# jpreprocess/jbonsai

Measured on AMD Instinct MI355X. Metric: 48 kHz PCM samples/sec (whole node), batched utterances, higher is better.
Workload: dtype f64

## Files before the change

### include/jbonsai_amd.h

```cpp
#ifndef JBONSAI_AMD_H
#define JBONSAI_AMD_H

#include <stddef.h>
#include <stdint.h>

#ifdef __cplusplus
extern "C" {
#endif

#define JB_MAX_STREAM 3
#define JB_MAX_WINDOW 8
#define JB_NODATA (-1e10)

typedef enum jb_status {
    JB_OK = 0,
    JB_ERR_INVALID = -1,
    JB_ERR_UNSUPPORTED = -2,
    JB_ERR_DEVICE = -3,
    JB_ERR_MODEL = -4,
    JB_ERR_LABEL = -5,
    JB_ERR_PARSE_OPTION = -6,
    JB_ERR_WEIGHT = -7,
    JB_ERR_BUFFER = -8
} jb_status;
// ... 94 lines not shown
int jb_batch_create_indexed(const jb_voice_desc *voice, const jb_pdf_set *set, const jb_index_utt *utts,
                            size_t n_utts, const jb_batch_opts *opts, jb_batch **out);
typedef struct jb_utt_voc {
    double alpha, beta, volume;
} jb_utt_voc;
int jb_batch_create_voc(const jb_voice_desc *voice, const jb_state_utt *utts, size_t n_utts, const jb_utt_voc *voc,
                        const jb_batch_opts *opts, jb_batch **out);
int jb_batch_create_indexed_voc(const jb_voice_desc *voice, const jb_pdf_set *set, const jb_index_utt *utts,
                                size_t n_utts, const jb_utt_voc *voc, const jb_batch_opts *opts, jb_batch **out);
int jb_batch_run(jb_batch *b);
int jb_batch_sync(jb_batch *b);
int jb_batch_run_timed(jb_batch *b, float *total_ms, float *vocoder_ms);
int jb_batch_last_timing(jb_batch *b, float *total_ms, float *vocoder_ms);
size_t jb_batch_size(const jb_batch *b);
size_t jb_batch_num_frames(const jb_batch *b, size_t utt);
size_t jb_batch_num_samples(const jb_batch *b, size_t utt);
size_t jb_batch_total_samples(const jb_batch *b);
int jb_batch_read_pcm(jb_batch *b, size_t utt, double *dst, size_t cap);
int jb_batch_read_pcm_i16(jb_batch *b, size_t utt, int16_t *dst, size_t cap);
int jb_batch_read_pcm_all(jb_batch *b, double *const *dst);
int jb_batch_read_pcm_i16_all(jb_batch *b, int16_t *const *dst);
int jb_batch_read_track(jb_batch *b, size_t utt, uint32_t stream, double *dst, size_t cap);
int jb_release_cached_memory(void);
int jb_set_cached_memory_limit(size_t megabytes);
int jb_batch_read_coefficients(jb_batch *b, size_t utt, double *dst, size_t cap);
int jb_batch_read_first_coefficients(jb_batch *b, size_t utt, double *dst, size_t cap);
int jb_batch_read_excitation(jb_batch *b, size_t utt, double *dst, size_t cap);
void *jb_batch_device_pcm(jb_batch *b, size_t *n_samples);
size_t jb_batch_pcm_offset(const jb_batch *b, size_t utt);
int jb_batch_info(const jb_batch *b, uint32_t *chunk_frames, uint32_t *warmup_frames,
                  uint32_t *n_items, uint32_t *n_redo);
int jb_batch_redo_stats(const jb_batch *b, uint32_t *n_partial, uint32_t *n_full);
int jb_batch_kernel_info(const jb_batch *b, uint32_t *lane_triple, uint32_t *waves_per_simd);
uint32_t jb_batch_gang_fallbacks(const jb_batch *b);
int jb_batch_set_output_rate(jb_batch *b, const uint32_t *out_hz, size_t n);
uint32_t jb_batch_output_rate(const jb_batch *b, size_t utt);
int jb_batch_read_pcm_native(jb_batch *b, size_t utt, double *dst, size_t cap);
int jb_batch_set_loudness_target(jb_batch *b, const double *target_lufs, size_t n, double ceiling_dbfs);
int jb_batch_loudness(jb_batch *b, size_t utt, double *lufs, double *peak_dbfs, double *gain_db);
void jb_batch_free(jb_batch *b);

int jb_paramgen_vocode_batch(const jb_voice_desc *voice, const jb_state_utt *utts, size_t n_utts,
                             const jb_batch_opts *opts, double *const *pcm, size_t *n_samples);

int jb_mlpg_batch(const jb_voice_desc *voice, const jb_state_utt *utts, size_t n_utts, const jb_batch_opts *opts,
                  double *const *tracks, size_t *n_frames);

typedef struct jb_track_utt {
    size_t n_spectrum, n_lf0, n_lpf;
    uint32_t spectrum_width, lf0_width, lpf_width;
    uint32_t reserved;
    const double *spectrum;
    const double *lf0;
    const double *lpf;
} jb_track_utt;
int jb_batch_create_from_tracks(const jb_voice_desc *voice, const jb_track_utt *utts, size_t n_utts,
                                const jb_batch_opts *opts, jb_batch **out);
int jb_vocode_tracks_batch(const jb_voice_desc *voice, const jb_track_utt *utts, size_t n_utts,
                           const jb_batch_opts *opts, double *const *pcm, size_t *n_samples);
int jb_vocoder_synthesize_batch(const jb_voice_desc *voice, const jb_track_utt *utts, size_t n_utts,
                                const jb_batch_opts *opts, double *const *pcm, size_t *n_samples);

int jb_resample_filter(uint32_t in_hz, uint32_t out_hz, uint32_t *L, uint32_t *M, uint32_t *ntaps, double *taps,
                       size_t cap);
int jb_resample_pcm_batch(const double *const *in, const size_t *n_in, size_t n, uint32_t in_hz, uint32_t out_hz,
                          int32_t device, double **out, size_t *n_out);
// ... 162 lines not shown
```

### jbonsai_amd/_ffi.py

```python
from __future__ import annotations

import ctypes as C
import subprocess
from pathlib import Path

_HERE = Path(__file__).resolve().parent
LIB_PATH = _HERE / "libjbonsai_amd.so"

MAX_STREAM = 3
MAX_WINDOW = 8
NODATA = -1e10

JB_OK = 0
ERRORS = {
    -1: "JB_ERR_INVALID", -2: "JB_ERR_UNSUPPORTED", -3: "JB_ERR_DEVICE", -4: "JB_ERR_MODEL",
    -5: "JB_ERR_LABEL", -6: "JB_ERR_PARSE_OPTION", -7: "JB_ERR_WEIGHT", -8: "JB_ERR_BUFFER",
}
BATCH_KEEP_TRACKS = 1
BATCH_GENERIC_MLPG = 2
BATCH_SERIAL = 4
BATCH_WAVE_KERNEL = 8
BATCH_LANE_KERNEL = 16
BATCH_SERIAL_GV = 32
BATCH_PCM_I16 = 64
# ... 75 lines not shown


class IndexUtt(C.Structure):
    _fields_ = [
        ("num_states", C.c_uint32),
        ("durations", C.POINTER(C.c_uint32)),
        ("stream", IndexStream * MAX_STREAM),
        ("lf0_offset", C.c_double),
    ]


class TrackUtt(C.Structure):
    _fields_ = [
        ("n_spectrum", C.c_size_t), ("n_lf0", C.c_size_t), ("n_lpf", C.c_size_t),
        ("spectrum_width", C.c_uint32), ("lf0_width", C.c_uint32), ("lpf_width", C.c_uint32),
        ("reserved", C.c_uint32),
        ("spectrum", C.POINTER(C.c_double)), ("lf0", C.POINTER(C.c_double)), ("lpf", C.POINTER(C.c_double)),
    ]


class UttVoc(C.Structure):
    _fields_ = [("alpha", C.c_double), ("beta", C.c_double), ("volume", C.c_double)]


class BatchOpts(C.Structure):
    _fields_ = [("device", C.c_int32), ("flags", C.c_uint32), ("chunk_frames", C.c_uint32),
                ("warmup_frames", C.c_uint32), ("verify_tol", C.c_double), ("reserved0", C.c_uint32), ("reserved", C.c_uint32)]


SYMBOLS = [
    "jb_batch_create", "jb_batch_run", "jb_batch_sync", "jb_batch_run_timed", "jb_batch_last_timing", "jb_batch_size",
    "jb_batch_num_frames", "jb_batch_num_samples", "jb_batch_total_samples", "jb_batch_read_pcm",
    "jb_batch_read_pcm_i16", "jb_batch_read_pcm_all", "jb_batch_read_pcm_i16_all", "jb_pdf_set_create", "jb_pdf_set_free", "jb_batch_create_indexed", "jb_batch_read_track", "jb_release_cached_memory", "jb_set_cached_memory_limit", "jb_batch_read_coefficients", "jb_batch_read_first_coefficients", "jb_batch_read_excitation", "jb_batch_device_pcm", "jb_batch_pcm_offset",
    "jb_batch_info", "jb_batch_kernel_info", "jb_batch_redo_stats", "jb_batch_gang_fallbacks", "jb_batch_free", "jb_paramgen_vocode_batch",
    "jb_mlpg_batch", "jb_batch_create_from_tracks", "jb_vocode_tracks_batch",
    "jb_engine_load", "jb_engine_load_from_bytes", "jb_engine_new", "jb_engine_free",
    "jb_engine_set_sampling_frequency", "jb_engine_get_sampling_frequency",
    "jb_engine_set_fperiod", "jb_engine_get_fperiod", "jb_engine_set_volume", "jb_engine_get_volume",
    "jb_engine_set_msd_threshold", "jb_engine_get_msd_threshold", "jb_engine_set_gv_weight",
    "jb_engine_get_gv_weight", "jb_engine_set_phoneme_alignment_flag",
    "jb_engine_get_phoneme_alignment_flag", "jb_engine_set_batch_invariant", "jb_engine_get_batch_invariant",
    "jb_engine_set_fast_invariant", "jb_engine_get_fast_invariant",
    "jb_engine_set_speed", "jb_engine_get_speed",
    "jb_engine_set_alpha", "jb_engine_get_alpha", "jb_engine_set_beta", "jb_engine_get_beta",
    "jb_engine_set_additional_half_tone", "jb_engine_get_additional_half_tone",
    "jb_engine_num_voices", "jb_engine_num_streams", "jb_engine_num_states",
    "jb_engine_set_interpolation_weight", "jb_engine_get_interpolation_weight", "jb_synthesize", "jb_pcm_free", "jb_write_wav_i16", "jb_write_wav_f64", "jb_synthesize_batch", "jb_synthesize_batch_i16", "jb_pcm_i16_free",
    "jb_engine_model_shape", "jb_engine_pdf_table", "jb_engine_tree_index",
    "jb_engine_states", "jb_states_utt", "jb_engine_voice_desc", "jb_states_free",
    "jb_generator_new", "jb_generator_new_from_tracks", "jb_vocoder_synthesize_batch", "jb_generator_fperiod", "jb_generator_synthesized_frames",
    "jb_generator_total_frames", "jb_generator_step", "jb_generator_step_n", "jb_generator_free",
    "jb_comm_unique_id", "jb_comm_init", "jb_comm_rank", "jb_comm_size", "jb_comm_free", "jb_gather_pcm",
    "jb_gathered_samples", "jb_gathered_sample_bytes", "jb_gathered_device", "jb_gathered_read", "jb_gathered_free",
    "jb_lpt_partition", "jb_paramgen_vocode_batch_multi", "jb_synthesize_batch_multi", "jb_synthesize_batch_i16_multi",
    "jb_states_duration_params", "jb_last_error", "jb_device_count", "jb_device_arch", "jb_device_pci_bus_id", "jb_version", "jb_default_verify_tol",
    "jb_batch_create_voc", "jb_batch_create_indexed_voc", "jb_synthesize_batch_each", "jb_synthesize_batch_each_i16",
    "jb_batch_set_output_rate", "jb_batch_output_rate", "jb_batch_read_pcm_native", "jb_resample_filter",
    "jb_resample_pcm_batch", "jb_engine_set_output_sampling_frequency", "jb_engine_get_output_sampling_frequency",
    "jb_batch_set_loudness_target", "jb_batch_loudness", "jb_loudness_filter", "jb_loudness_pcm_batch",
    "jb_engine_set_loudness_target", "jb_engine_get_loudness_target", "jb_engine_set_peak_ceiling",
    "jb_engine_get_peak_ceiling",
]


def build(force: bool = False) -> Path:
    srcs = list((_HERE / "csrc").glob("*.hip")) + list((_HERE / "csrc").glob("*.cpp")) + \
        list((_HERE / "csrc").glob("*.h")) + [_HERE.parent / "include" / "jbonsai_amd.h"]
# ... 27 lines not shown
                                  C.POINTER(vp)]
    L.jb_pdf_set_create.argtypes = [C.POINTER(PdfTable), C.c_uint32, C.c_uint32, C.c_int32, C.POINTER(vp)]
    L.jb_pdf_set_free.argtypes = [vp]
    L.jb_pdf_set_free.restype = None
    L.jb_batch_create_indexed.argtypes = [C.POINTER(VoiceDesc), vp, C.POINTER(IndexUtt), sz, C.POINTER(BatchOpts),
                                          C.POINTER(vp)]
    L.jb_batch_create_voc.argtypes = [C.POINTER(VoiceDesc), C.POINTER(StateUtt), sz, C.POINTER(UttVoc),
                                      C.POINTER(BatchOpts), C.POINTER(vp)]
    L.jb_batch_create_indexed_voc.argtypes = [C.POINTER(VoiceDesc), vp, C.POINTER(IndexUtt), sz, C.POINTER(UttVoc),
                                              C.POINTER(BatchOpts), C.POINTER(vp)]
    L.jb_batch_run.argtypes = [vp]
    L.jb_batch_sync.argtypes = [vp]
    L.jb_batch_run_timed.argtypes = [vp, C.POINTER(C.c_float), C.POINTER(C.c_float)]
    L.jb_batch_last_timing.argtypes = [vp, C.POINTER(C.c_float), C.POINTER(C.c_float)]
    for n in ("jb_batch_size", "jb_batch_total_samples"):
        getattr(L, n).restype = sz
        getattr(L, n).argtypes = [vp]
    for n in ("jb_batch_num_frames", "jb_batch_num_samples", "jb_batch_pcm_offset"):
        getattr(L, n).restype = sz
        getattr(L, n).argtypes = [vp, sz]
    L.jb_batch_read_pcm.argtypes = [vp, sz, vp, sz]
    L.jb_batch_read_pcm_all.argtypes = [vp, C.POINTER(vp)]
    L.jb_batch_read_pcm_i16_all.argtypes = [vp, C.POINTER(vp)]
    L.jb_batch_read_track.argtypes = [vp, sz, C.c_uint32, vp, sz]
    L.jb_batch_read_coefficients.argtypes = [vp, sz, vp, sz]
    L.jb_batch_read_first_coefficients.argtypes = [vp, sz, vp, sz]
    L.jb_batch_read_pcm_i16.argtypes = [vp, sz, vp, sz]
    L.jb_batch_read_excitation.argtypes = [vp, sz, vp, sz]
    L.jb_batch_device_pcm.restype = vp
    L.jb_batch_device_pcm.argtypes = [vp, C.POINTER(sz)]
    L.jb_batch_info.argtypes = [vp] + [C.POINTER(C.c_uint32)] * 4
    L.jb_batch_redo_stats.argtypes = [vp, C.POINTER(C.c_uint32), C.POINTER(C.c_uint32)]
    L.jb_batch_kernel_info.argtypes = [vp, C.POINTER(C.c_uint32), C.POINTER(C.c_uint32)]
    L.jb_batch_gang_fallbacks.argtypes = [vp]
    L.jb_batch_gang_fallbacks.restype = C.c_uint32
    L.jb_batch_free.argtypes = [vp]
    L.jb_batch_free.restype = None
    L.jb_paramgen_vocode_batch.argtypes = [C.POINTER(VoiceDesc), C.POINTER(StateUtt), sz,
                                           C.POINTER(BatchOpts), C.POINTER(dp), C.POINTER(sz)]
    L.jb_mlpg_batch.argtypes = [C.POINTER(VoiceDesc), C.POINTER(StateUtt), sz, C.POINTER(BatchOpts),
                                C.POINTER(dp), C.POINTER(sz)]
    L.jb_batch_create_from_tracks.argtypes = [C.POINTER(VoiceDesc), C.POINTER(TrackUtt), sz, C.POINTER(BatchOpts),
                                              C.POINTER(vp)]
    L.jb_vocode_tracks_batch.argtypes = [C.POINTER(VoiceDesc), C.POINTER(TrackUtt), sz, C.POINTER(BatchOpts),
                                         C.POINTER(dp), C.POINTER(sz)]
    L.jb_vocoder_synthesize_batch.argtypes = [C.POINTER(VoiceDesc), C.POINTER(TrackUtt), sz, C.POINTER(BatchOpts),
                                              C.POINTER(dp), C.POINTER(sz)]
    L.jb_generator_new_from_tracks.argtypes = [C.POINTER(VoiceDesc), C.POINTER(TrackUtt), C.POINTER(BatchOpts),
                                               C.POINTER(vp)]
    L.jb_set_cached_memory_limit.argtypes = [sz]
    L.jb_comm_unique_id.argtypes = [C.c_char_p, sz]
    L.jb_comm_init.argtypes = [C.c_char_p, C.c_int, C.c_int, C.c_int32, C.POINTER(vp)]
    L.jb_comm_rank.argtypes = [vp]
    L.jb_comm_size.argtypes = [vp]
    L.jb_comm_free.argtypes = [vp]
    L.jb_comm_free.restype = None
    L.jb_gather_pcm.argtypes = [vp, vp, C.c_int, C.POINTER(vp), C.POINTER(C.c_float)]
    L.jb_gathered_samples.argtypes = [vp, C.c_int]
    L.jb_gathered_samples.restype = sz
    L.jb_gathered_sample_bytes.argtypes = [vp]
    L.jb_gathered_sample_bytes.restype = sz
    L.jb_gathered_device.argtypes = [vp, C.c_int]
    L.jb_gathered_device.restype = vp
    L.jb_gathered_read.argtypes = [vp, C.c_int, vp, sz]
    L.jb_gathered_free.argtypes = [vp]
    L.jb_gathered_free.restype = None
# ... 101 lines not shown
```

### jbonsai_amd/batch.py

```python
from __future__ import annotations

import ctypes as C
from dataclasses import dataclass, field
from typing import List, Optional, Sequence

import numpy as np

from . import _ffi as F


def _dp(a):
    return a.ctypes.data_as(C.POINTER(C.c_double)) if a is not None else None


@dataclass
class StreamInfo:
    vector_length: int
    is_msd: bool
    use_gv: bool
    windows: List[List[float]]


@dataclass
class VoiceInfo:
# ... 233 lines not shown
            F.check(L.jb_batch_create(C.byref(vd), arr, len(utts), C.byref(opts), C.byref(h)))
        self._h = h
        self._keep = keep

    def __len__(self):
        return self._L.jb_batch_size(self._h)

    def run(self):
        F.check(self._L.jb_batch_run(self._h))

    def sync(self):
        F.check(self._L.jb_batch_sync(self._h))

    def run_timed(self):
        t, v = C.c_float(), C.c_float()
        F.check(self._L.jb_batch_run_timed(self._h, C.byref(t), C.byref(v)))
        return t.value, v.value

    def last_timing(self):
        t, v = C.c_float(), C.c_float()
        F.check(self._L.jb_batch_last_timing(self._h, C.byref(t), C.byref(v)))
        return t.value, v.value

    def info(self):
        v = [C.c_uint32() for _ in range(4)]
        F.check(self._L.jb_batch_info(self._h, *[C.byref(x) for x in v]))
        return dict(chunk_frames=v[0].value, warmup_frames=v[1].value, n_items=v[2].value, n_redo=v[3].value)

    def kernel_info(self):
        lt, w = C.c_uint32(), C.c_uint32()
        F.check(self._L.jb_batch_kernel_info(self._h, C.byref(lt), C.byref(w)))
        return ("k_vocoder_lt" if lt.value else "k_vocoder"), w.value

    def num_samples(self, i):
        return self._L.jb_batch_num_samples(self._h, i)

    def num_frames(self, i):
        return self._L.jb_batch_num_frames(self._h, i)

    @property
    def total_samples(self):
        return self._L.jb_batch_total_samples(self._h)

    def pcm(self, i) -> np.ndarray:
        n = self.num_samples(i)
        out = np.empty(n, dtype=np.float64)
        F.check(self._L.jb_batch_read_pcm(self._h, i, out.ctypes.data, n))
        return out

    def pcm_i16(self, i) -> np.ndarray:
        n = self.num_samples(i)
        out = np.empty(n, dtype=np.int16)
        F.check(self._L.jb_batch_read_pcm_i16(self._h, i, out.ctypes.data, n))
        return out

    def pcm_all(self, out: Optional[List[np.ndarray]] = None) -> List[np.ndarray]:
        i16 = bool(self.flags & F.BATCH_PCM_I16)
        dt = np.int16 if i16 else np.float64
        n = len(self)
        if out is None:
            out = [np.empty(self.num_samples(i), dtype=dt) for i in range(n)]
        ptrs = (C.c_void_p * max(1, n))(*[o.ctypes.data if o.size else None for o in out])
        fn = self._L.jb_batch_read_pcm_i16_all if i16 else self._L.jb_batch_read_pcm_all
        F.check(fn(self._h, ptrs))
        return out

# ... 172 lines not shown
```

### jbonsai_amd/csrc/jb_batch.cpp

```cpp
#include "jb_host.h"

#include <algorithm>
#include <atomic>
#include <chrono>
#include <cmath>
#include <cstdlib>
#include <cstring>
#include <map>
#include <new>
#include <set>
#include <tuple>
#include <numeric>
#include <thread>

namespace jb {

thread_local std::string g_err;

void set_error(const std::string &s) { g_err = s; }

int hip_fail(hipError_t e, const char *what)
{
    set_error(std::string(what) + ": " + hipGetErrorString(e));
    return JB_ERR_DEVICE;
// ... 1236 lines not shown
    if ((rc = b->build_work(opts)))
        return rc;
    if ((rc = b->flush_zero()))
        return rc;
    if ((rc = b->flush_uploads()))
        return rc;
    for (auto &c : b->up_chunks)
        c.host.reset();
    cmark("work list built");
    e = hipStreamSynchronize(nullptr);
    if (e == hipSuccess)
        e = hipStreamSynchronize(b->stream);
    if (e != hipSuccess)
        return hip_fail(e, "upload");
    cmark("synchronised");
    *out = b.release();
    return JB_OK;
}

int Batch::build_work(const jb_batch_opts *opts)
{
    verify_tol = (opts && opts->verify_tol > 0.0) ? opts->verify_tol : kDefaultVerifyTol;
    VocPlanIn in;
    in.T = T.data();
    in.B = (size_t)B;
    in.first_of_kind = first_of_kind.empty() ? nullptr : first_of_kind.data();
    in.voc_class = uvoc.empty() ? nullptr : voc_class.data();
    in.nmcp = vd.nmcp;
    in.fperiod = vd.fperiod;
    in.stage = vd.stage;
    in.flags = flags;
    in.chunk_frames = opts ? opts->chunk_frames : 0;
    in.warmup_frames = opts ? opts->warmup_frames : 0;
    const VocPlan plan = plan_vocoder_work(in);
    lp_mode = plan.lane_kernel;
    lt_waves_per_simd = plan.waves_per_simd;
    chunk_frames = plan.chunk_frames;
    warmup_frames = plan.warmup_frames;
    vd.ckpt_frames = plan.ckpt_frames;
    vd.ckpt2_frames = plan.ckpt2_frames;
    n_items = (uint32_t)plan.items.size();
    int rc;
    if ((rc = dalloc(&bad_dev, n_items, true)) ||
        (rc = dalloc(&nbad_dev, 1, true)))
        return rc;
    const int stride = vd.state_stride;
    if (chunk_frames != 0) {
        if ((rc = dalloc(&end_state, (size_t)n_items * stride, true)) ||
            (rc = dalloc(&warm_state, (size_t)n_items * stride, true)) ||
            (rc = dalloc(&ckpt_state, (size_t)n_items * stride, true)) ||
            (vd.ckpt2_frames && (rc = dalloc(&ckpt2_state, (size_t)n_items * stride, true))))
            return rc;
        state_stride = stride;
    }
    work.resize(n_items);
    for (uint32_t k = 0; k < n_items; k++) {
        const VocPlanItem &it = plan.items[k];
        auto slot = [&](double *states, uint8_t bit) { return (it.saves & bit) ? states + (size_t)k * stride : nullptr; };
        work[k] = VocWork{it.utt, it.t_start, it.t_out, it.t_end, nullptr, slot(warm_state, kSaveWarm),
                          slot(end_state, kSaveEnd), slot(ckpt_state, kSaveCkpt), slot(ckpt2_state, kSaveCkpt2)};
    }
    if ((rc = stage(work.data(), n_items, &work_dev)))
        return rc;
    if (lp_mode) {
        n_slots = (uint32_t)plan.order.size();
        if ((rc = stage(plan.order.data(), plan.order.size(), &order_dev)))
            return rc;
    }
    return JB_OK;
}

int Batch::build_generator_work()
{
// ... 1414 lines not shown
        return JB_OK;
    return b->read(b->vd.exc + (size_t)b->frame_off[i] * b->voice.fperiod, dst, ns * sizeof(double));
}

int jb_batch_info(const jb_batch *hb, uint32_t *chunk_frames, uint32_t *warmup_frames,
                  uint32_t *n_items, uint32_t *n_redo)
{
    const Batch *b = (const Batch *)hb;
    if (!b)
        return JB_ERR_INVALID;
    if (chunk_frames)
        *chunk_frames = b->chunk_frames;
    if (warmup_frames)
        *warmup_frames = b->warmup_frames;
    if (n_items)
        *n_items = b->n_items;
    if (n_redo)
        *n_redo = b->n_redo;
    return JB_OK;
}

int jb_batch_kernel_info(const jb_batch *hb, uint32_t *lane_triple, uint32_t *waves_per_simd)
{
    const Batch *b = (const Batch *)hb;
    if (!b)
        return JB_ERR_INVALID;
    if (lane_triple)
        *lane_triple = b->lp_mode ? 1u : 0u;
    if (waves_per_simd)
        *waves_per_simd = b->lp_mode ? (uint32_t)b->lt_waves_per_simd : 0u;
    return JB_OK;
}

int jb_batch_redo_stats(const jb_batch *hb, uint32_t *n_partial, uint32_t *n_full)
{
    const Batch *b = (const Batch *)hb;
    if (!b)
        return JB_ERR_INVALID;
    if (n_partial)
        *n_partial = b->n_redo_partial;
    if (n_full)
        *n_full = b->n_redo_full;
    return JB_OK;
}

uint32_t jb_batch_gang_fallbacks(const jb_batch *b) { return b ? ((const Batch *)b)->gang_fallbacks : 0; }

void jb_batch_free(jb_batch *b) { delete (Batch *)b; }

int jb_paramgen_vocode_batch(const jb_voice_desc *voice, const jb_state_utt *utts, size_t n,
                             const jb_batch_opts *opts, double *const *pcm, size_t *n_samples)
{
    jb_batch *hb = nullptr;
    int rc = jb_batch_create(voice, utts, n, opts, &hb);
    if (rc)
        return rc;
    std::unique_ptr<Batch> guard((Batch *)hb);
    if (n_samples)
        for (size_t i = 0; i < n; i++)
            n_samples[i] = jb_batch_num_samples(hb, i);
    if (!pcm)
        return JB_OK;
    if ((rc = guard->run(false)) || (rc = guard->sync()))
        return rc;
    for (size_t i = 0; i < n; i++) {
        size_t ns = jb_batch_num_samples(hb, i);
// ... 89 lines not shown
```

### jbonsai_amd/csrc/jb_device.h

```cpp
#pragma once
#include "jb_plan.h"

#include <hip/hip_runtime.h>
#include <stdint.h>
#include <vector>

namespace jb {

constexpr int kMaxStream = 3;
constexpr int kMaxWin = 8;
constexpr int kMaxCoef = 32;
constexpr int kMaxBand = 9;
constexpr int kPade = 5;
constexpr int kGroups = 12;
constexpr int kMaxTPL = 6;
constexpr int kMaxNmcp = 64;
constexpr double kNoData = -1e10;

struct StreamStatesDev {
    const double *mean;
    const double *var;
    const double *msd;
    const double *gv_mean;
    const double *gv_var;
// ... 106 lines not shown
    double beta_stage;
    double *bfirst;
    double *pf_table;
    uint32_t n_pf;
    double *pf_rcp;
    double *pitch;
    double *cur_start;
    double *pinc;
    unsigned long long *pmask;
    const uint8_t *voiced;
    const uint32_t *run_list;
    const uint32_t *nruns;
    uint32_t *run_base;
    uint32_t *run_counter;
    const double *noise;
    uint64_t noise_len;
    double *xin;
    int skip_unvoiced;
    double *exc_tab;
    const uint8_t *lpf_canon;
    int lpf_sparse;
    uint8_t *exc_src;
    uint32_t *exc_gen;
    uint32_t *exc_gen_count;
    int exc_no_table;
    uint32_t *uv_before;
    double *pcm;
    int16_t *pcm16;
    double *exc;
    double *state;
    int state_stride;
    uint32_t ckpt_frames;
    uint32_t ckpt2_frames;
};

__device__ __forceinline__ double voc_alpha(const VocDev &vd, uint32_t b)
{
    return vd.uvoc ? vd.uvoc[b].alpha : vd.alpha;
}
__device__ __forceinline__ double voc_volume(const VocDev &vd, uint32_t b)
{
    return vd.uvoc ? vd.uvoc[b].volume : vd.volume;
}
__device__ __forceinline__ double voc_beta_stage(const VocDev &vd, uint32_t b)
{
    return vd.uvoc ? vd.uvoc[b].beta_stage : vd.beta_stage;
}
__device__ __forceinline__ double wave_uniform(double v)
{
    const int lo = __builtin_amdgcn_readfirstlane(__double2loint(v));
    const int hi = __builtin_amdgcn_readfirstlane(__double2hiint(v));
    return __hiloint2double(hi, lo);
}
__device__ __forceinline__ uint32_t wave_uniform(uint32_t v) { return (uint32_t)__builtin_amdgcn_readfirstlane((int)v); }

__device__ __forceinline__ const double *lpf_row(const VocDev &vd, uint64_t f, int NL)
{
    return vd.lpf + ((vd.lpf_sparse && vd.lpf_canon[f]) ? 0ull : f) * (uint64_t)NL;
}

__device__ __forceinline__ uint32_t exc_code(const VocDev &vd, uint64_t base, uint32_t t)
{
    if (vd.exc_src)
        return vd.exc_src[base + t];
    return (vd.skip_unvoiced && t >= 1 && !vd.voiced[base + t] && !vd.voiced[base + t - 1]) ? 1u : 0u;
}
// ... 104 lines not shown
```

### jbonsai_amd/csrc/jb_plan.cpp

```cpp
#include "jb_plan.h"

#include "../../include/jbonsai_amd.h"

#include <algorithm>
#include <numeric>

namespace jb {
namespace {

uint32_t inv_chunk(uint32_t Ti)
{
    constexpr uint32_t kInvChunks = 96, kInvMin = 16, kInvMax = 153;
    return std::min(std::max((Ti + kInvChunks - 1) / kInvChunks, kInvMin), kInvMax);
}

}

VocPlan plan_vocoder_work(const VocPlanIn &in)
{
    VocPlan p;
    const bool serial = (in.flags & JB_BATCH_SERIAL) != 0;
    const bool invariant = (in.flags & JB_BATCH_INVARIANT) && !serial;
    uint64_t sumT = 0;
    for (size_t i = 0; i < in.B; i++)
// ... 31 lines not shown
        ch = 0;
    } else if (ch == 0 && p.lane_kernel) {
        constexpr uint64_t cfloor = 16;
        auto launch_cost = [&](uint64_t slots, double us_per_sample) {
            return (double)(std::max<uint64_t>((sumT + slots - 1) / slots, cfloor) + p.warmup_frames) * us_per_sample;
        };
        if (!warmup_given)
            p.warmup_frames = warmup_at(std::max<uint64_t>((sumT + 2 * slots1 - 1) / (2 * slots1), cfloor));
        p.waves_per_simd = launch_cost(slots1, 0.90) < launch_cost(2 * slots1, 1.42) ? 1 : 2;
        const uint64_t target = slots1 * (uint64_t)p.waves_per_simd;
        uint64_t c = (sumT + target - 1) / target;
        constexpr uint64_t cmin = cfloor;
        ch = (uint32_t)std::max<uint64_t>(c, cmin);
        for (int guard = 0; guard < 256 && c >= cmin && chunks_at(ch) > target; guard++)
            ch += 1;
        if (p.waves_per_simd == 1 && chunks_at(ch) > slots1)
            p.waves_per_simd = 2;
    } else if (ch == 0) {
        const uint64_t target = sumT >= 400000 ? 2048 : 1024;
        const uint64_t floor_w = sumT < 1024 ? 6 : sumT < 8192 ? 8 : 16;
        ch = (uint32_t)std::max<uint64_t>((sumT + target - 1) / target, floor_w);
        if (ch >= 16)
            ch = (ch + 7) / 8 * 8;
    }
    p.chunk_frames = ch;
    if (!warmup_given && ch != 0 && !invariant)
        p.warmup_frames = warmup_at(ch);
    if (p.lane_kernel && ch != 0 && in.chunk_frames)
        p.waves_per_simd = chunks_at(ch) <= slots1 ? 1 : 2;
    p.ckpt_frames = invariant ? kVocCkptFrames
                    : ch >= 2 * kVocCkptFrames ? kVocCkptFrames
                    : ch >= kVocCkptFramesShort + 12 ? kVocCkptFramesShort
                    : ch >= kVocCkptFramesTiny + 8 ? kVocCkptFramesTiny : 0;
    p.ckpt2_frames = invariant || (p.ckpt_frames == kVocCkptFrames && ch >= kVocCkpt2Frames + 48) ? kVocCkpt2Frames : 0;
    const uint32_t need = p.ckpt_frames + (p.ckpt_frames < kVocCkptFramesShort ? 8u : 12u);
    for (size_t i = 0; i < in.B; i++) {
        const uint32_t Ti = in.T[i];
        if (Ti == 0)
            continue;
        const uint32_t ci = invariant ? inv_chunk(Ti) : ch;
        if (ci == 0 || Ti <= ci + p.warmup_frames) {
            p.items.push_back(VocPlanItem{(uint32_t)i, 0, 0, Ti, 0});
            continue;
        }
        for (uint32_t t0 = 0; t0 < Ti; t0 += ci) {
            VocPlanItem w{(uint32_t)i, t0 > p.warmup_frames ? t0 - p.warmup_frames : 0, t0, std::min(Ti, t0 + ci), 0};
            const bool first = t0 == 0;
            w.saves = kSaveEnd;
            if (!first)
                w.saves |= kSaveWarm;
            if (!first && p.ckpt_frames && w.t_end - w.t_out >= need)
                w.saves |= kSaveCkpt;
            if ((w.saves & kSaveCkpt) && p.ckpt2_frames && w.t_end - w.t_out >= p.ckpt2_frames + 12u)
                w.saves |= kSaveCkpt2;
            p.items.push_back(w);
        }
    }
    if (ch == 0)
        std::stable_sort(p.items.begin(), p.items.end(), [](const VocPlanItem &a, const VocPlanItem &c) {
            return (a.t_end - a.t_start) > (c.t_end - c.t_start);
        });
    if (p.lane_kernel) {
        const uint32_t n = (uint32_t)p.items.size();
        auto len = [&](uint32_t k) { return p.items[k].t_end - p.items[k].t_start; };
        std::vector<uint32_t> ord(n);
        std::iota(ord.begin(), ord.end(), 0u);
// ... 22 lines not shown
```

### jbonsai_amd/csrc/jb_plan.h

```cpp
#pragma once
#include <stddef.h>
#include <stdint.h>
#include <vector>

namespace jb {

constexpr int lt_code_nm(int nmcp)
{
    return nmcp <= 25 ? 25 : nmcp <= 31 ? 31 : nmcp <= 35 ? 35
         : nmcp <= 41 ? 41 : nmcp <= 51 ? 51 : nmcp <= 61 ? 61 : 0;
}
constexpr int lt_chunks(int lpc) { return lpc == 3 ? 21 : 12; }
constexpr bool vocoder_ls_supported(int nmcp) { return nmcp >= 7 && lt_code_nm(nmcp) != 0; }
constexpr int vocoder_ls_chunks_per_wave(int nmcp) { return lt_chunks(lt_code_nm(nmcp) <= 35 ? 3 : 5); }
constexpr uint32_t kLtNoItem = 0xffffffffu;

constexpr uint32_t kVocCkptFrames = 48, kVocCkptFramesShort = 24, kVocCkptFramesTiny = 16, kVocCkpt2Frames = 96;

struct VocPlanIn {
    const uint32_t *T = nullptr;
    size_t B = 0;
    const uint8_t *first_of_kind = nullptr;
    const uint32_t *voc_class = nullptr;
    int nmcp = 0, fperiod = 0, stage = 0;
    uint32_t flags = 0;
    uint32_t chunk_frames = 0, warmup_frames = 0;
};

enum : uint8_t { kSaveEnd = 1, kSaveWarm = 2, kSaveCkpt = 4, kSaveCkpt2 = 8 };

struct VocPlanItem {
    uint32_t utt, t_start, t_out, t_end;
    uint8_t saves;
};

struct VocPlan {
    bool lane_kernel = false;
    int waves_per_simd = 2;
    uint32_t chunk_frames = 0;
    uint32_t warmup_frames = 0;
    uint32_t ckpt_frames = 0, ckpt2_frames = 0;
    std::vector<VocPlanItem> items;
    std::vector<uint32_t> order;
};

VocPlan plan_vocoder_work(const VocPlanIn &in);

}
```

### jbonsai_amd/csrc/jb_vocoder.hip

```cpp
#include "jb_device.h"

#include <cstdlib>
#include <cstring>

namespace jb {

__global__ void k_pitch(BatchDev bd, VocDev vd)
{
    const int b = blockIdx.y;
    const UttDev *u = bd.utt + b;
    const uint32_t t = blockIdx.x * blockDim.x + threadIdx.x;
    if (t >= u->T)
        return;
    const uint64_t f = u->frame_off + t;
    const double MAX_LF0 = 9.903487552536127, MIN_LF0 = 2.995732273553991;
    auto pitch_of = [&](double l) {
        if (l == kNoData)
            return 0.0;
        const double cl = l < MIN_LF0 ? MIN_LF0 : (l > MAX_LF0 ? MAX_LF0 : l);
        return (double)vd.fs / exp(cl);
    };
    const double p = pitch_of(vd.lf0[f]);
    const double prevp = t > 0 ? pitch_of(vd.lf0[f - 1]) : 0.0;
    vd.pitch[f] = p;
// ... 1427 lines not shown
                x += v1;
                double out = v5;
                out += v4;
                out += v3;
                out += v2;
                out += v1;
                ulane = fma(hmask, dpp_f64<DPP_WAVE_SHR1>(Y), l0mask * x);
                x += out;
#pragma unroll
                for (int k = 0; k < TPL; k++)
                    cd[k] += cdinc[k];
                if (lane == 0)
                    os[i] = x;
            }
            if (++q == nblk) {
                q = 0;
                t++;
            }
        }
        __syncthreads();
    }
    if (NB && wk.save_end)
        save_state(wk.save_end);
}

constexpr int DPP_WAVE_SHL1 = 0x130;
constexpr int DPP_ROW_SHL1 = 0x101, DPP_ROW_SHL2 = 0x102, DPP_ROW_SHL4 = 0x104;
__device__ __forceinline__ double fold5(double s)
{
    const double t1 = s + dpp_f64<DPP_ROW_SHL1>(s);
    const double t2 = t1 + dpp_f64<DPP_ROW_SHL2>(t1);
    return t2 + dpp_f64<DPP_ROW_SHL4>(s);
}
constexpr int kLtPf = 4;
constexpr int kLtBalance = 8;
#ifdef JB_LT_STAMPS
constexpr unsigned kLtStampWaves = 4096;
__device__ unsigned long long g_lt_stamp[kLtStampWaves][4];
#endif
#ifdef JB_LT_CLOCKS
__device__ unsigned long long g_lt_clk[8];
#endif

template <int NM, int TPLW_, int kLtWaves, bool EXACT = true, int LPC = 3>
__global__ __launch_bounds__(64 * kLtWaves, 2) void k_vocoder_lt(BatchDev bd, VocDev vd,
                                                       const VocWork *__restrict__ work,
                                                       const uint32_t *__restrict__ order,
                                                       uint32_t n_items)
{
    static_assert(LPC == 3 || LPC == 5, "three lanes x two stage slots, or five lanes x one");
    constexpr int M = NM - 1;
    constexpr int NS = LPC == 3 ? 2 : 1;
    constexpr int kLtChunks = lt_chunks(LPC);
    const int nm = EXACT ? NM : vd.nmcp;
    const int mreal = nm - 1;
    const int TPLW = EXACT ? TPLW_ : (mreal + kGroups - 1) / kGroups;
    const int lane = threadIdx.x % 64;
    const int wv = threadIdx.x / 64;
    const bool idle = LPC == 3 ? lane == 63 : (lane & 15) == 15;
    const int pos = LPC == 3 ? (idle ? 2 : lane % 3) : (idle ? 4 : (lane & 15) % 5);
    const int ci = LPC == 3 ? (idle ? 20 : lane / 3) : (lane >> 4) * 3 + (idle ? 2 : (lane & 15) / 5);
    const uint32_t slot = (blockIdx.x * (uint32_t)kLtWaves + (uint32_t)wv) * (uint32_t)kLtChunks + (uint32_t)ci;
    const uint32_t oslot = (!idle && slot < n_items) ? order[slot] : kLtNoItem;
    const bool has = oslot != kLtNoItem;
    const bool lead = has && pos == 0;
    const uint32_t item = has ? oslot : 0u;
    struct {
        uint32_t utt, t_start, t_out, t_end;
        const double *load_state;
    } wk = {0, 0, 0, 0, nullptr};
    if (has) {
        const VocWork &w0 = work[item];
        wk.utt = w0.utt;
        wk.t_start = w0.t_start;
        wk.t_out = w0.t_out;
        wk.t_end = w0.t_end;
        wk.load_state = w0.load_state;
    }
    const uint32_t T = has ? bd.utt[wk.utt].T : 0;
    if (wk.t_end > T)
        wk.t_end = T;
    const uint32_t nfr = wk.t_end > wk.t_start ? wk.t_end - wk.t_start : 0;
    uint32_t maxfr = nfr;
    for (int o = 32; o > 0; o >>= 1)
        maxfr = max(maxfr, (uint32_t)__shfl_xor((int)maxfr, o));
    __shared__ uint32_t prog[8];
    if (kLtWaves == 8 && lane == 0)
        prog[wv] = maxfr == 0 ? 0xffffffffu : 0u;
    if (maxfr == 0)
        return;
#ifdef JB_LT_STAMPS
    const unsigned stamp_w = blockIdx.x * (unsigned)kLtWaves + (unsigned)wv;
    if (lane == 0 && stamp_w < kLtStampWaves) {
        unsigned hw, xcc;
        asm volatile("s_getreg_b32 %0, hwreg(HW_REG_HW_ID)" : "=s"(hw));
        asm volatile("s_getreg_b32 %0, hwreg(HW_REG_XCC_ID, 0, 4)" : "=s"(xcc));
        g_lt_stamp[stamp_w][0] = wall_clock64();
        g_lt_stamp[stamp_w][2] = (unsigned long long)hw | ((unsigned long long)xcc << 32);
        g_lt_stamp[stamp_w][3] = maxfr;
    }
#endif
#ifdef JB_LT_CLOCKS
    const int clk_slot = wv != 0 ? -1 : blockIdx.x == 0 ? 0 : blockIdx.x == gridDim.x / 2 ? 4 : -1;
    if (clk_slot >= 0 && lane == 0) {
        g_lt_clk[clk_slot] = clock64();
        g_lt_clk[clk_slot + 1] = wall_clock64();
    }
#endif
    const uint64_t base = has ? bd.utt[wk.utt].frame_off : 0;
    const int fp = vd.fperiod;
    double a = vd.alpha, vol = vd.volume;
    if (vd.uvoc) {
        const uint32_t u0 = wave_uniform(wk.utt);
        a = wave_uniform(vd.uvoc[u0].alpha);
        vol = wave_uniform(vd.uvoc[u0].volume);
    }
    const double na = -a, iaa = 1.0 - a * a;
    const int s0 = NS * pos;
    const double w0 = kPPade[s0 + 1];
    const double w1 = (NS == 2 && s0 + 1 < kPade) ? kPPade[s0 + 2] : 0.0;
    const double wa = (NS == 1 && (pos & 1)) ? -w0 : w0;

    __shared__ double2 cc_[kLtWaves][NM - 1][kLtChunks];
    __shared__ double gqs_[kLtWaves][kLtChunks];
    double2 (*const cc)[kLtChunks] = cc_[wv];
    double *const gqs = gqs_[wv];
#define JB_LT_FENCE() asm volatile("s_waitcnt lgkmcnt(0)" ::: "memory")

    if (!EXACT && has)
        for (int k = nm + pos; k < NM; k += LPC)
            cc[k - 1][ci] = make_double2(0.0, 0.0);
    double d[NS][M + 1];
    double u[NS];
    double gain = 1.0;
    double e11[NS], e12[NS], ein = 0.0;
#pragma unroll
    for (int q = 0; q < NS; q++) {
        e11[q] = e12[q] = 0.0;
        u[q] = 0.0;
#pragma unroll
        for (int j = 0; j <= M; j++)
            d[q][j] = 0.0;
    }

    auto layout_tpl = [&]() {
        int tp = TPLW;
        if (!EXACT)
            asm volatile("" : "+s"(tp));
        return tp;
    };
    if (wk.load_state) {
        const double *sp = wk.load_state;
        const int tpl = layout_tpl();
#pragma unroll
        for (int q = 0; q < NS; q++) {
            const int st = s0 + q;
            if (st < kPade) {
                u[q] = sp[64 * tpl + kGroups * st];
                int kk = 0, gg = 0;
#pragma unroll
                for (int j = 1; j <= M; j++) {
                    if (EXACT)
                        d[q][j] = sp[64 * ((j - 1) % TPLW_) + kGroups * st + (j - 1) / TPLW_];
                    else if (j <= mreal)
                        d[q][j] = sp[64 * kk + kGroups * st + gg];
                    if (++kk == tpl) {
                        kk = 0;
                        gg++;
                    }
                }
            }
        }
#pragma unroll
        for (int q = 0; q < NS; q++) {
            const int st = s0 + 1 + q;
// ... 670 lines not shown
```

Before: 20.26 billion.

## Run vocoder warmup head frames in packed f32 before the f64 loop

Adds a packed-f32 pre-pass in the lane vocoder kernel that runs most of each chunk's warmup frames (up to a tail margin) in single precision. It then converts the filter state to f64 and continues the exact loop from there. The aim is to cut the cost of the f64 warmup recursion, which only settles filter state and whose output is discarded. The risk is small state error carried into the exact region, and extra code and register pressure. The head length is set by the planner and can be overridden by an environment variable.

```diff
diff --git a/include/jbonsai_amd.h b/include/jbonsai_amd.h
--- a/include/jbonsai_amd.h
+++ b/include/jbonsai_amd.h
@@ -150,6 +150,7 @@
                   uint32_t *n_items, uint32_t *n_redo);
 int jb_batch_redo_stats(const jb_batch *b, uint32_t *n_partial, uint32_t *n_full);
 int jb_batch_kernel_info(const jb_batch *b, uint32_t *lane_triple, uint32_t *waves_per_simd);
+uint32_t jb_batch_voc_head_frames(const jb_batch *b);
 uint32_t jb_batch_gang_fallbacks(const jb_batch *b);
 int jb_batch_set_output_rate(jb_batch *b, const uint32_t *out_hz, size_t n);
 uint32_t jb_batch_output_rate(const jb_batch *b, size_t utt);
diff --git a/jbonsai_amd/_ffi.py b/jbonsai_amd/_ffi.py
--- a/jbonsai_amd/_ffi.py
+++ b/jbonsai_amd/_ffi.py
@@ -131,7 +131,7 @@
     "jb_batch_create", "jb_batch_run", "jb_batch_sync", "jb_batch_run_timed", "jb_batch_last_timing", "jb_batch_size",
     "jb_batch_num_frames", "jb_batch_num_samples", "jb_batch_total_samples", "jb_batch_read_pcm",
     "jb_batch_read_pcm_i16", "jb_batch_read_pcm_all", "jb_batch_read_pcm_i16_all", "jb_pdf_set_create", "jb_pdf_set_free", "jb_batch_create_indexed", "jb_batch_read_track", "jb_release_cached_memory", "jb_set_cached_memory_limit", "jb_batch_read_coefficients", "jb_batch_read_first_coefficients", "jb_batch_read_excitation", "jb_batch_device_pcm", "jb_batch_pcm_offset",
-    "jb_batch_info", "jb_batch_kernel_info", "jb_batch_redo_stats", "jb_batch_gang_fallbacks", "jb_batch_free", "jb_paramgen_vocode_batch",
+    "jb_batch_info", "jb_batch_kernel_info", "jb_batch_voc_head_frames", "jb_batch_redo_stats", "jb_batch_gang_fallbacks", "jb_batch_free", "jb_paramgen_vocode_batch",
     "jb_mlpg_batch", "jb_batch_create_from_tracks", "jb_vocode_tracks_batch",
     "jb_engine_load", "jb_engine_load_from_bytes", "jb_engine_new", "jb_engine_free",
     "jb_engine_set_sampling_frequency", "jb_engine_get_sampling_frequency",
@@ -225,6 +225,8 @@
     L.jb_batch_info.argtypes = [vp] + [C.POINTER(C.c_uint32)] * 4
     L.jb_batch_redo_stats.argtypes = [vp, C.POINTER(C.c_uint32), C.POINTER(C.c_uint32)]
     L.jb_batch_kernel_info.argtypes = [vp, C.POINTER(C.c_uint32), C.POINTER(C.c_uint32)]
+    L.jb_batch_voc_head_frames.argtypes = [vp]
+    L.jb_batch_voc_head_frames.restype = C.c_uint32
     L.jb_batch_gang_fallbacks.argtypes = [vp]
     L.jb_batch_gang_fallbacks.restype = C.c_uint32
     L.jb_batch_free.argtypes = [vp]
diff --git a/jbonsai_amd/batch.py b/jbonsai_amd/batch.py
--- a/jbonsai_amd/batch.py
+++ b/jbonsai_amd/batch.py
@@ -289,6 +289,9 @@
         F.check(self._L.jb_batch_kernel_info(self._h, C.byref(lt), C.byref(w)))
         return ("k_vocoder_lt" if lt.value else "k_vocoder"), w.value
 
+    def voc_head_frames(self):
+        return self._L.jb_batch_voc_head_frames(self._h)
+
     def num_samples(self, i):
         return self._L.jb_batch_num_samples(self._h, i)
 
diff --git a/jbonsai_amd/csrc/jb_batch.cpp b/jbonsai_amd/csrc/jb_batch.cpp
--- a/jbonsai_amd/csrc/jb_batch.cpp
+++ b/jbonsai_amd/csrc/jb_batch.cpp
@@ -1292,6 +1292,8 @@
     in.flags = flags;
     in.chunk_frames = opts ? opts->chunk_frames : 0;
     in.warmup_frames = opts ? opts->warmup_frames : 0;
+    if (const char *ev = getenv("JB_VOC_F32_HEAD"))
+        in.head_frames = std::max(0, atoi(ev));
     const VocPlan plan = plan_vocoder_work(in);
     lp_mode = plan.lane_kernel;
     lt_waves_per_simd = plan.waves_per_simd;
@@ -1299,6 +1301,8 @@
     warmup_frames = plan.warmup_frames;
     vd.ckpt_frames = plan.ckpt_frames;
     vd.ckpt2_frames = plan.ckpt2_frames;
+    vd.lt_head_frames = plan.head_frames;
+    vd.lt_head_warm = plan.warmup_frames;
     n_items = (uint32_t)plan.items.size();
     int rc;
     if ((rc = dalloc(&bad_dev, n_items, true)) ||
@@ -2779,6 +2783,8 @@
     return JB_OK;
 }
 
+uint32_t jb_batch_voc_head_frames(const jb_batch *b) { return b ? ((const Batch *)b)->vd.lt_head_frames : 0; }
+
 int jb_batch_redo_stats(const jb_batch *hb, uint32_t *n_partial, uint32_t *n_full)
 {
     const Batch *b = (const Batch *)hb;
diff --git a/jbonsai_amd/csrc/jb_device.h b/jbonsai_amd/csrc/jb_device.h
--- a/jbonsai_amd/csrc/jb_device.h
+++ b/jbonsai_amd/csrc/jb_device.h
@@ -162,6 +162,7 @@
     int state_stride;
     uint32_t ckpt_frames;
     uint32_t ckpt2_frames;
+    uint32_t lt_head_frames, lt_head_warm;
 };
 
 __device__ __forceinline__ double voc_alpha(const VocDev &vd, uint32_t b)
diff --git a/jbonsai_amd/csrc/jb_plan.cpp b/jbonsai_amd/csrc/jb_plan.cpp
--- a/jbonsai_amd/csrc/jb_plan.cpp
+++ b/jbonsai_amd/csrc/jb_plan.cpp
@@ -87,6 +87,11 @@
                     : ch >= 2 * kVocCkptFrames ? kVocCkptFrames
                     : ch >= kVocCkptFramesShort + 12 ? kVocCkptFramesShort
                     : ch >= kVocCkptFramesTiny + 8 ? kVocCkptFramesTiny : 0;
+    if (p.lane_kernel && ch != 0 && lt_code_nm(in.nmcp) <= 35) {
+        const uint32_t cap = p.warmup_frames > kVocHeadTailMin ? p.warmup_frames - kVocHeadTailMin : 0;
+        const uint32_t def = p.warmup_frames > kVocHeadTail ? p.warmup_frames - kVocHeadTail : 0;
+        p.head_frames = in.head_frames < 0 ? def : std::min<uint32_t>((uint32_t)in.head_frames, cap);
+    }
     p.ckpt2_frames = invariant || (p.ckpt_frames == kVocCkptFrames && ch >= kVocCkpt2Frames + 48) ? kVocCkpt2Frames : 0;
     const uint32_t need = p.ckpt_frames + (p.ckpt_frames < kVocCkptFramesShort ? 8u : 12u);
     for (size_t i = 0; i < in.B; i++) {
diff --git a/jbonsai_amd/csrc/jb_plan.h b/jbonsai_amd/csrc/jb_plan.h
--- a/jbonsai_amd/csrc/jb_plan.h
+++ b/jbonsai_amd/csrc/jb_plan.h
@@ -15,6 +15,7 @@
 constexpr int vocoder_ls_chunks_per_wave(int nmcp) { return lt_chunks(lt_code_nm(nmcp) <= 35 ? 3 : 5); }
 constexpr uint32_t kLtNoItem = 0xffffffffu;
 
+constexpr uint32_t kVocHeadTail = 14, kVocHeadTailMin = 2;
 constexpr uint32_t kVocCkptFrames = 48, kVocCkptFramesShort = 24, kVocCkptFramesTiny = 16, kVocCkpt2Frames = 96;
 
 struct VocPlanIn {
@@ -25,6 +26,7 @@
     int nmcp = 0, fperiod = 0, stage = 0;
     uint32_t flags = 0;
     uint32_t chunk_frames = 0, warmup_frames = 0;
+    int head_frames = -1;
 };
 
 enum : uint8_t { kSaveEnd = 1, kSaveWarm = 2, kSaveCkpt = 4, kSaveCkpt2 = 8 };
@@ -40,6 +42,7 @@
     uint32_t chunk_frames = 0;
     uint32_t warmup_frames = 0;
     uint32_t ckpt_frames = 0, ckpt2_frames = 0;
+    uint32_t head_frames = 0;
     std::vector<VocPlanItem> items;
     std::vector<uint32_t> order;
 };
diff --git a/jbonsai_amd/csrc/jb_vocoder.hip b/jbonsai_amd/csrc/jb_vocoder.hip
--- a/jbonsai_amd/csrc/jb_vocoder.hip
+++ b/jbonsai_amd/csrc/jb_vocoder.hip
@@ -1483,6 +1483,11 @@
     const double t2 = t1 + dpp_f64<DPP_ROW_SHL2>(t1);
     return t2 + dpp_f64<DPP_ROW_SHL4>(s);
 }
+template <int CTRL>
+__device__ __forceinline__ float dpp_f32(float v)
+{
+    return __int_as_float(__builtin_amdgcn_update_dpp(0, __float_as_int(v), CTRL, 0xf, 0xf, true));
+}
 constexpr int kLtPf = 4;
 constexpr int kLtBalance = 8;
 #ifdef JB_LT_STAMPS
@@ -1531,7 +1536,11 @@
     const uint32_t T = has ? bd.utt[wk.utt].T : 0;
     if (wk.t_end > T)
         wk.t_end = T;
-    const uint32_t nfr = wk.t_end > wk.t_start ? wk.t_end - wk.t_start : 0;
+    uint32_t nfr = wk.t_end > wk.t_start ? wk.t_end - wk.t_start : 0;
+    const uint32_t hl = LPC == 3 && has && !wk.load_state && vd.lt_head_frames &&
+                                wk.t_out - wk.t_start >= vd.lt_head_warm && nfr > vd.lt_head_frames
+                            ? vd.lt_head_frames : 0u;
+    const uint32_t hw = LPC == 3 && __ballot(hl != 0) ? wave_uniform(vd.lt_head_frames) : 0u;
     uint32_t maxfr = nfr;
     for (int o = 32; o > 0; o >>= 1)
         maxfr = max(maxfr, (uint32_t)__shfl_xor((int)maxfr, o));
@@ -1592,6 +1601,116 @@
 #pragma unroll
         for (int j = 0; j <= M; j++)
             d[q][j] = 0.0;
+    }
+
+    if constexpr (LPC == 3) {
+        if (hw) {
+            typedef float v2f __attribute__((ext_vector_type(2)));
+            constexpr int NP = M / 2;
+            const float af = (float)a, iaaf = (float)iaa;
+            const v2f a2 = {af, af}, na2 = {-af, -af}, iaa2 = {iaaf, iaaf};
+            const float w0f = (float)w0, w1f = (float)w1;
+            v2f df[M + 1];
+#pragma unroll
+            for (int j = 1; j <= M; j++)
+                df[j] = v2f{0.0f, 0.0f};
+            v2f uf = {0.0f, 0.0f}, e11f = {0.0f, 0.0f}, e12f = {0.0f, 0.0f};
+            float einf = 0.0f;
+            for (uint32_t tl = 0; tl < hw; tl++) {
+                const uint32_t t = wk.t_start + (hl ? tl : 0u);
+                const uint64_t f = base + t;
+                v2f c0[NP], ci[NP];
+                float gainf, gqf;
+                {
+                    const double *bcur = vd.bcoef + f * (uint64_t)nm;
+                    const double *bprev = (t > 0) ? bcur - nm : (vd.bfirst ? vd.bfirst + (uint64_t)wk.utt * nm : bcur);
+#pragma unroll
+                    for (int p = 0; p < NP; p++) {
+                        float c0p[2], cip[2];
+#pragma unroll
+                        for (int h = 0; h < 2; h++) {
+                            const int k = 2 * p + 1 + h;
+                            const double c0v = EXACT || k < nm ? bprev[k] : 0.0, c1v = EXACT || k < nm ? bcur[k] : 0.0;
+                            c0p[h] = (float)c0v;
+                            cip[h] = (float)((c1v - c0v) / (double)fp);
+                        }
+                        c0[p] = v2f{c0p[0], c0p[1]};
+                        ci[p] = v2f{cip[0], cip[1]};
+                    }
+                    gainf = (float)exp(bprev[0]);
+                    gqf = (float)exp((bcur[0] - bprev[0]) / (double)fp);
+                }
+                const uint32_t xcode = hl ? exc_code(vd, base, t) : 1u;
+                const int xbs = vd.bs;
+                auto xblock = [&](int q) -> const double * { return hl ? exc_block_ptr(vd, base, t, xcode, q) : vd.noise; };
+                const double *xq = xblock(0);
+                int xnext = xbs, xqn = 1;
+                double xn = xq[0];
+                for (int i = 0; i < fp; i++) {
+                    float x = (float)xn * gainf;
+                    gainf *= gqf;
+                    if (i + 1 == xnext && xnext < fp) {
+                        xq = xblock(xqn);
+                        xqn++;
+                        xnext += xbs;
+                    }
+                    if (i + 1 < fp)
+                        xn = xq[i + 1];
+                    const float fi = (float)i;
+                    const v2f fi2 = {fi, fi};
+                    v2f cv = __builtin_elementwise_fma(fi2, ci[0], c0[0]);
+                    {
+                        const v2f ein2 = {einf, e12f.x};
+                        e11f = __builtin_elementwise_fma(iaa2, ein2, a2 * e11f);
+                        e12f = e11f * cv.xx;
+                    }
+                    const float dv1 = w1f * e12f.y;
+                    const float da = fmaf(w0f, e12f.x, -dv1);
+                    const float db1 = fmaf(w0f, e12f.x, dv1);
+                    x += da + dpp_f32<DPP_WAVE_SHL1>(da + dpp_f32<DPP_WAVE_SHL1>(da));
+                    const float eprev = dpp_f32<DPP_WAVE_SHR1>(e12f.y);
+                    einf = pos == 0 ? x : eprev;
+                    v2f r = uf, y = {0.0f, 0.0f};
+#pragma unroll
+                    for (int j = 1; j <= M; j++) {
+                        if (j > 2 && (j & 1))
+                            cv = __builtin_elementwise_fma(fi2, ci[(j - 1) / 2], c0[(j - 1) / 2]);
+                        const v2f rn = __builtin_elementwise_fma(na2, r, df[j]);
+                        df[j] = __builtin_elementwise_fma(a2, rn, r);
+                        r = rn;
+                        if (j == 2)
+                            y = cv.yy * df[j];
+                        else if (j > 2)
+                            y = __builtin_elementwise_fma((j & 1) ? cv.xx : cv.yy, df[j], y);
+                    }
+                    const float v1 = w1f * y.y;
+                    const float sa = fmaf(w0f, y.x, db1 - v1);
+                    const float ssum = sa + dpp_f32<DPP_WAVE_SHL1>(sa + dpp_f32<DPP_WAVE_SHL1>(sa));
+                    const float yprev = dpp_f32<DPP_WAVE_SHR1>(y.y);
+                    const float xmid = x + ssum;
+                    uf = v2f{pos == 0 ? xmid : yprev, y.x};
+                }
+            }
+            if (hl) {
+#pragma unroll
+                for (int j = 1; j <= M; j++) {
+                    d[0][j] = (double)df[j].x;
+                    d[1][j] = (double)df[j].y;
+                }
+                u[0] = (double)uf.x;
+                u[1] = (double)uf.y;
+                e11[0] = (double)e11f.x;
+                e11[1] = (double)e11f.y;
+                e12[0] = (double)e12f.x;
+                e12[1] = (double)e12f.y;
+                ein = (double)einf;
+            }
+            wk.t_start += hl;
+            nfr -= hl;
+            maxfr = nfr;
+            for (int o = 32; o > 0; o >>= 1)
+                maxfr = max(maxfr, (uint32_t)__shfl_xor((int)maxfr, o));
+        }
     }
 
     auto layout_tpl = [&]() {
```

Result: faster. 20.51 billion (median of 6 runs) (+1.2%).
